# redmod-team/SympGPR

Hardware: AMD Instinct MI355X
Metric: Gram-build GB/s + Cholesky fp64 TFLOP/s at N=65536 d=2; |alpha-alpha_ref|/|alpha_ref| (higher is better)
Workload: dtype f64

## Files before the change

include/sympgpr_probe.h:

```cpp
#ifndef SYMPGPR_PROBE_H
#define SYMPGPR_PROBE_H
#include <stddef.h>
#ifdef __cplusplus
extern "C" {
#endif

int sgpr_probe_mfma_f64(int waves_per_simd, int iters, double *tflops);
int sgpr_probe_hbm_write(size_t bytes, int reps, double *gbs);
int sgpr_probe_mfma_clock(int nacc, int waves_per_simd, int iters, double *out3);
int sgpr_probe_gemm(int m, int n, int k, int lower, double *out4);
int sgpr_probe_gemm_debug(int bits);
int sgpr_probe_leaf(double *out8);
int sgpr_probe_lat(double *out8);
int sgpr_probe_xcc(int nblocks, int *host_out);
int sgpr_probe_cumask(const unsigned *mask_words, int nwords, int nblocks, int *host_out);

int sgpr_probe_generated_eval(int family, int which, int m, const double *xa, const double *ya,
                              const double *xb, const double *yb, const double *l, int nl, double *out);

int sgpr_probe_queue_plan(int n, int nworkers, int *starts_out, int max_starts, unsigned *tasks_out, int max_tasks,
                          int *counts);
int sgpr_probe_queue_plan_partial(int n, int nworkers, int nq, int *starts_out, int max_starts, unsigned *tasks_out,
                                  int max_tasks, int *counts);
int sgpr_probe_queue_trace_begin(int max_tasks);
int sgpr_probe_queue_trace_end(unsigned long long *out, int max_tasks);
int sgpr_probe_queue_trace_clear(void);
int sgpr_probe_queue_postmortem(int always);
int sgpr_probe_queue_force_giveup(int on);
int sgpr_probe_tune(const char *name, double value);
unsigned sgpr_probe_map_calls(void);
int sgpr_probe_map_team(int ntest, int n0);

int sgpr_probe_trsm_piece(int ticket, int cap, int strips, int out[5]);
int sgpr_probe_trsm_counts(int strips, int cap, unsigned long long out[2]);

int sgpr_probe_census(int na, int threads_a, int lds_a, int spin_a, const unsigned *mask_a, int nwords_a,
                      int nb, int threads_b, int lds_b, int spin_b, const unsigned *mask_b, int nwords_b,
                      unsigned long long *host_out);

#ifdef __cplusplus
}
#endif
#endif
```

sympgpr_amd/_lib.py:

```python
import ctypes as C
import os

import numpy as np

FAMILIES = {"A": 0, "B": 1, "C": 2, "D": 3, "USER": 4}
K_KERN, K_DXDX0, K_DYDY0, K_DXDY0 = 0, 1, 2, 3
K_DLX, K_DLY = 4, 8
K_DX, K_DY, K_DX0, K_DY0, K_DXDX0DY0, K_DYDY0DY0, K_DXDY0DY0 = 16, 17, 18, 19, 20, 21, 22
G_QQ, G_PQ, G_QP, G_PP, G_ALL, G_LOWER, G_OCML, G_DLX, G_DLY = 1, 2, 4, 8, 15, 16, 32, 64, 128
FIT_LOWER_ONLY, FIT_REG, FIT_BLOCK_QQ, FIT_BLOCK_PP = 1, 4, 8, 16
MAP_WRAP_Q, MAP_WRAP_P, MAP_EXPLICIT, MAP_LOSS_NEGP = 1, 2, 4, 8
E_ARG, E_NODEVICE, E_HIP, E_NOMEM, E_STATE = -1, -2, -3, -4, -5

ABI_VERSION = 5
_dp = C.POINTER(C.c_double)
_vp = C.c_void_p


class SympGPRError(RuntimeError):
    pass


class NoDeviceError(SympGPRError):
    pass
# ... 108 lines not shown
    "sgpr_probe_generated_eval": (C.c_int, [C.c_int, C.c_int, C.c_int, _dp, _dp, _dp, _dp, _dp, C.c_int, _dp]),
    "sgpr_probe_queue_plan": (C.c_int, [C.c_int, C.c_int, C.POINTER(C.c_int), C.c_int, C.POINTER(C.c_uint), C.c_int,
                                        C.POINTER(C.c_int)]),
    "sgpr_probe_queue_plan_partial": (C.c_int, [C.c_int, C.c_int, C.c_int, C.POINTER(C.c_int), C.c_int, C.POINTER(C.c_uint),
                                                C.c_int, C.POINTER(C.c_int)]),
    "sgpr_probe_queue_trace_begin": (C.c_int, [C.c_int]),
    "sgpr_probe_queue_trace_end": (C.c_int, [C.POINTER(C.c_ulonglong), C.c_int]),
    "sgpr_probe_queue_postmortem": (C.c_int, [C.c_int]),
    "sgpr_probe_queue_force_giveup": (C.c_int, [C.c_int]),
    "sgpr_probe_tune": (C.c_int, [C.c_char_p, C.c_double]),
    "sgpr_probe_map_calls": (C.c_uint, []),
    "sgpr_probe_map_team": (C.c_int, [C.c_int, C.c_int]),
    "sgpr_probe_trsm_piece": (C.c_int, [C.c_int, C.c_int, C.c_int, C.POINTER(C.c_int)]),
    "sgpr_probe_trsm_counts": (C.c_int, [C.c_int, C.c_int, C.POINTER(C.c_ulonglong)]),
    "sgpr_probe_queue_trace_clear": (C.c_int, []),
    "sgpr_probe_census": (C.c_int, [C.c_int, C.c_int, C.c_int, C.c_int, C.POINTER(C.c_uint), C.c_int,
                                    C.c_int, C.c_int, C.c_int, C.c_int, C.POINTER(C.c_uint), C.c_int,
                                    C.POINTER(C.c_ulonglong)]),
}

_LIB = None
_PROBE = None


def load_library():
    global _LIB
    if _LIB is not None:
        return _LIB
    path = lib_path()
    if os.environ.get("SYMPGPR_NO_TORCH_PRELOAD") != "1":
# ... 81 lines not shown
```

sympgpr_amd/csrc/chol.hip:

```cpp
#include <algorithm>
#include <cstdlib>
#include <mutex>
#include <vector>

#include "cholq.h"
#include "common.h"
#include "gemm_tile.h"
#include "leaf.h"

namespace sgpr {

namespace {

using namespace leaf;


__global__ __launch_bounds__(LT) void leaf_kernel(int nb, double *A, size_t lda, double *inv,
                                                  int *dinfo, int goff, int mode,
                                                  unsigned long long *stamps)
{
    __shared__ double s[LEAF_LDS];
    if (nb == LEAF) leaf_body(s, (int)LEAF, A, lda, inv, dinfo, goff, mode, stamps);
    else            leaf_body(s, nb, A, lda, inv, dinfo, goff, mode, stamps);
}
// ... 759 lines not shown

inline int split(int n)
{
    int n1 = ((n / 2 + LEAF - 1) / LEAF) * LEAF;
    if (n1 >= n) n1 -= LEAF;
    return n1;
}

struct Ctx {
    double *inv;
    int *dinfo;
    hipStream_t st;
    int la_max = 0;
    int *flags = nullptr;
    void *qws = nullptr;
};

int potrf_lookahead(int n, double *A, size_t lda, const Ctx &c, int nb, int off0);
inline int la_block(int n) { return n <= 4096 ? 256 : (n <= 24576 ? 512 : (n <= 40960 ? 1024 : 2048)); }

int trsm_rec(int m, int n, const double *L, size_t ldl, double *B, size_t ldb, int off, const Ctx &c)
{
    if (n <= LEAF) {
        return gemm_nt(m, n, n, 1.0, B, ldb, c.inv + (size_t)(off / LEAF) * LEAF * LEAF, LEAF, 0.0,
                       B, ldb, 0, 0, c.st);
    }
    const int n1 = split(n), n2 = n - n1;
    int rc = trsm_rec(m, n1, L, ldl, B, ldb, off, c);
    if (rc) return rc;
    rc = gemm_nt(m, n2, n1, -1.0, B, ldb, L + n1, ldl, 1.0, B + (size_t)n1 * ldb, ldb, 0, 0, c.st);
    if (rc) return rc;
    return trsm_rec(m, n2, L + n1 + (size_t)n1 * ldl, ldl, B + (size_t)n1 * ldb, ldb, off + n1, c);
}

int trsm_rl_rec(int m, int n, const double *L, size_t ldl, double *B, size_t ldb, int off, const Ctx &c)
{
    if (n <= LEAF)
        return gemm_nn(m, n, n, 1.0, B, ldb, c.inv + (size_t)(off / LEAF) * LEAF * LEAF, LEAF, 0.0, B, ldb, c.st);
    const int n1 = split(n), n2 = n - n1;
    int rc = trsm_rl_rec(m, n2, L + n1 + (size_t)n1 * ldl, ldl, B + (size_t)n1 * ldb, ldb, off + n1, c);
    if (rc) return rc;
    rc = gemm_nn(m, n1, n2, -1.0, B + (size_t)n1 * ldb, ldb, L + n1, ldl, 1.0, B, ldb, c.st);
    if (rc) return rc;
    return trsm_rl_rec(m, n1, L, ldl, B, ldb, off, c);
}
// ... 2 lines not shown
{
    if (n <= LEAF) {
        hipLaunchKernelGGL(leaf_kernel, dim3(1), dim3(LT), 0, c.st, n, A, lda,
                           c.inv + (size_t)(off / LEAF) * LEAF * LEAF, c.dinfo, off, (int)LEAF_FACTOR,
                           (unsigned long long *)nullptr);
        SGPR_CHECK_LAUNCH();
        return 0;
    }
    if (n > 4 * LEAF && n <= c.la_max) return potrf_lookahead(n, A, lda, c, 0, off);
    const int n1 = split(n), n2 = n - n1;
    double *A21 = A + n1, *A22 = A + n1 + (size_t)n1 * lda;
    int rc = potrf_rec(n1, A, lda, off, c);
    if (rc) return rc;
    rc = trsm_rec(n2, n1, A, lda, A21, lda, off, c);
    if (rc) return rc;
    rc = gemm_nt(n2, n2, n1, -1.0, A21, lda, A21, lda, 1.0, A22, lda, 1, 0, c.st);
    if (rc) return rc;
    return potrf_rec(n2, A22, lda, off + n1, c);
}

int trsv_n_rec(int n, const double *L, size_t ldl, double *b, int off, const Ctx &c)
{
    if (n <= LEAF) {
        hipLaunchKernelGGL(leaf_matvec_kernel, dim3(1), dim3(MV_T), 0, c.st, n,
                           c.inv + (size_t)(off / LEAF) * LEAF * LEAF, b, 0);
        SGPR_CHECK_LAUNCH();
        return 0;
    }
    if (n <= TRSV_BLOCK) {
        hipLaunchKernelGGL(trsv_block_kernel, dim3(1), dim3(MV_T), 0, c.st, n, L, ldl,
                           c.inv + (size_t)(off / LEAF) * LEAF * LEAF, b, 0);
// ... 560 lines not shown
    QueueDevice &qd = g_qdev[dev];
    std::lock_guard<std::mutex> lock(qd.mu);
    qd.failed = true;
    return true;
}

int potrf_trim()
{
    for (int dev = 0; dev < 64; ++dev) {
        EventPool &p = t_event_pool[dev];
        if (p.ev.empty() || p.top != 0) continue;
        for (hipEvent_t e : p.ev) (void)hipEventDestroy(e);
        p.ev.clear();
    }
    (void)hipGetLastError();
    return 0;
}

int release_device_streams(int dev)
{
    if (dev < 0 || dev >= 64) { set_error("release_device_streams: device index out of range"); return SGPR_E_ARG; }
    return release_streams(dev);
}

int potrf(int n, double *A, size_t lda, void *work, size_t lwork, int *dinfo, hipStream_t st)
{
    if (n < 0 || (n > 0 && lda < (size_t)n)) { set_error("potrf: bad n / lda"); return SGPR_E_ARG; }
    if (lwork < potrf_workspace(n)) { set_error("potrf: workspace too small"); return SGPR_E_ARG; }
    SGPR_HIP(hipMemsetAsync(dinfo, 0, sizeof(int), st));
    if (n == 0) return 0;
    int *flags = reinterpret_cast<int *>(static_cast<char *>(work) + inv_bytes(n));
    SGPR_HIP(hipMemsetAsync(flags, 0, flag_bytes(n), st));
    static const int mode = [] { const char *e = getenv("SGPR_POTRF"); return !e ? 0 : (e[0] == 'r' ? 1 : 2); }();
    static const int nb_env = [] { const char *e = getenv("SGPR_POTRF_NB"); return e ? atoi(e) : 0; }();
    static const int la_max_env = [] { const char *e = getenv("SGPR_LA_MAX"); return e ? atoi(e) : 57344; }();
    t_last_potrf_used_queue = false;
    Ctx c{static_cast<double *>(work), dinfo, st, mode == 1 ? 0 : la_max_env, flags};
    if (cholq::ws_bytes(n) > 0) c.qws = static_cast<char *>(work) + inv_bytes(n) + flag_bytes(n) + pub_bytes(n);
    const bool dbg = PANEL_DBG && getenv("SGPR_PANEL_DBG") != nullptr;
    const int T = (n + LEAF - 1) / LEAF;
    if (dbg) {
        (void)hipMalloc((void **)&g_panel_dbg, sizeof(unsigned long long) * 16 * T);
        (void)hipMemset(g_panel_dbg, 0, sizeof(unsigned long long) * 16 * T);
    }
    int rc;
    if (mode == 2 || (nb_env > 0 && mode == 0 && n > 4 * LEAF && n <= c.la_max))
        rc = potrf_lookahead(n, A, lda, c, nb_env > 0 ? nb_env : 0, 0);
    else
        rc = potrf_rec(n, A, lda, 0, c);
    if (dbg) {
        (void)hipStreamSynchronize(st);
        std::vector<unsigned long long> h(16 * (size_t)T);
        (void)hipMemcpy(h.data(), g_panel_dbg, h.size() * 8, hipMemcpyDeviceToHost);
// ... 171 lines not shown
```

sympgpr_amd/csrc/common.h:

```cpp
#pragma once
#include <hip/hip_runtime.h>
#include <cstddef>
#include <cstdint>
#include <string>

#include "../../include/sympgpr_hip.h"

namespace sgpr {

void set_error(const std::string &msg);
double tune(const char *name, double dflt);
void tune_set(const char *name, double v);
int hip_fail(hipError_t e, const char *what, const char *file, int line);

#define SGPR_HIP(call)                                                          \
    do {                                                                        \
        hipError_t e__ = (call);                                                \
        if (e__ != hipSuccess) return ::sgpr::hip_fail(e__, #call, __FILE__, __LINE__); \
    } while (0)

#define SGPR_CHECK_LAUNCH() SGPR_HIP(hipGetLastError())

struct KConst {
    double lx, ly, p, sig;
// ... 37 lines not shown
            const double *hyp, int nhyp, double *K, size_t ld, size_t rstride, size_t cstride, long diag_off,
            double noise, hipStream_t st);
int gram_nd_sel(int family, int d, int mi, int mj, const double *Xb, size_t ldxb, const double *Xa, size_t ldxa,
                const double *hyp, int nhyp, double *K, size_t ld, const long *roff, const long *coff, hipStream_t st);
int predict_nd(int family, int d, int m, const double *Xt, size_t ldxt, int n0, const double *Xtr, size_t ldxtr,
               const double *hyp, int nhyp, const double *alpha, double *out, hipStream_t st);

int gemm_nt(int m, int n, int k, double alpha, const double *A, size_t lda, const double *B,
            size_t ldb, double beta, double *C, size_t ldc, int lower, long diag_off,
            hipStream_t st);
int gemm_nt_bc(int m, int n, int k, double alpha, const double *A, size_t lda, const double *B,
               size_t ldb, double beta, double *C, size_t ldc, int lower, const int *bc5,
               hipStream_t st);
int gemm_nn(int m, int n, int k, double alpha, const double *A, size_t lda, const double *B, size_t ldb,
            double beta, double *C, size_t ldc, hipStream_t st);
int gemm_profile_begin();
int gemm_profile_end(double *out12);
int gemm_profile_launches(double *buf, int max_records);
void gemm_set_overlap(int on);
int gemm_nt_diag(int m, int n, int k, double alpha, const double *A, size_t lda, const double *B, size_t ldb,
                 double beta, double *C, size_t ldc, int lower, unsigned long long *stamps, int dbg, hipStream_t st);

constexpr int LEAF = 128;
constexpr int POTRF_HANDOFF_TIMEOUT = -1000001;
constexpr int SOLVE_HANDOFF_TIMEOUT = -1000002;
inline int info_status(int info)
{
    if (info >= 0) return info;
    set_error(info == POTRF_HANDOFF_TIMEOUT ? "potrf: a hand-off inside the panel kernel timed out"
              : info == SOLVE_HANDOFF_TIMEOUT ? "solve: a hand-off between the strips of a triangular solve timed out" : "potrf: internal error");
// ... 87 lines not shown
```

sympgpr_amd/csrc/gemm_f64.hip:

```cpp
#include <algorithm>
#include <atomic>
#include <cstdlib>
#include <mutex>
#include <type_traits>
#include <vector>

#include "common.h"
#include "gemm_tile.h"

namespace sgpr {

namespace {

struct ProfRec { double flop; int big; int m, n, k, lower, overlap; };
struct Prof {
    std::mutex mu;
    std::atomic<bool> on{false};
    std::vector<hipEvent_t> pool;
    std::vector<ProfRec> recs;
    long dropped = 0;
};
constexpr int PROF_POOL = 8192;
Prof g_prof;
thread_local int t_overlap = 0;
// ... 15 lines not shown
    }
    const bool aligned = ((((uintptr_t)g.A | (uintptr_t)g.B) & 15) == 0) && (((g.lda | g.ldb) & 1) == 0);
    const bool fast = aligned && (row0 + BM <= g.m) && (col0 + BN <= g.n) && (g.k % BK == 0);
    if (g.transb) {
        if (fast) gemm_body<BM, BN, true, true>(g, smem, tile_r, tile_c);
        else      gemm_body<BM, BN, false, true>(g, smem, tile_r, tile_c);
        return;
    }
    if constexpr (BM % 128 == 0) {
        if (fast && !(g.dbg & 16)) { gemm_body_dma<BM, BN, STAGES>(g, smem, tile_r, tile_c); return; }
    }
    if (fast) gemm_body<BM, BN, true>(g, smem, tile_r, tile_c);
    else      gemm_body<BM, BN, false>(g, smem, tile_r, tile_c);
}

}

int gemm_nt(int m, int n, int k, double alpha, const double *A, size_t lda, const double *B,
            size_t ldb, double beta, double *C, size_t ldc, int lower, long diag_off,
            hipStream_t st)
{
    const int bc[5] = {1, 1, (int)diag_off, 1, 0};
    return gemm_nt_bc(m, n, k, alpha, A, lda, B, ldb, beta, C, ldc, lower, bc, st);
}

static int gemm_launch(int m, int n, int k, double alpha, const double *A, size_t lda, const double *B,
                       size_t ldb, double beta, double *C, size_t ldc, int lower, const int *bc, int transb,
                       hipStream_t st, unsigned long long *stamps = nullptr, int dbg = 0);

int gemm_nt_bc(int m, int n, int k, double alpha, const double *A, size_t lda, const double *B,
               size_t ldb, double beta, double *C, size_t ldc, int lower, const int *bc,
               hipStream_t st)
{
    static const int kmax = [] { const char *e = getenv("SGPR_GEMM_KMAX"); return e ? atoi(e) : 8192; }();
    if (kmax >= 128 && k > kmax) {
        const int nchunk = (k + kmax - 1) / kmax;
        const int step = ((k + nchunk - 1) / nchunk + 127) / 128 * 128;
        for (int k0 = 0; k0 < k; k0 += step) {
            const int rc = gemm_launch(m, n, std::min(step, k - k0), alpha, A + (size_t)k0 * lda, lda, B + (size_t)k0 * ldb, ldb,
                                       k0 == 0 ? beta : 1.0, C, ldc, lower, bc, 0, st);
            if (rc) return rc;
        }
        return 0;
    }
    return gemm_launch(m, n, k, alpha, A, lda, B, ldb, beta, C, ldc, lower, bc, 0, st);
}

static int gemm_launch(int m, int n, int k, double alpha, const double *A, size_t lda, const double *B,
                       size_t ldb, double beta, double *C, size_t ldc, int lower, const int *bc, int transb,
                       hipStream_t st, unsigned long long *stamps, int dbg)
{
    const bool plain = bc[0] == 1 && bc[1] == 1 && bc[3] == 1 && bc[4] == 0;
    const long diag_off = plain ? bc[2] : 1;
    if (bc[0] < 1 || bc[1] < 1 || bc[3] < 1) { set_error("gemm_nt: bad block-cyclic descriptor"); return SGPR_E_ARG; }
    if (m < 0 || n < 0 || k < 0) { set_error("gemm_nt: negative extent"); return SGPR_E_ARG; }
    if (m == 0 || n == 0) return 0;
    if (lda < (size_t)m || ldb < (size_t)(transb ? k : n) || ldc < (size_t)m) {
        set_error("gemm: leading dimension too small");
        return SGPR_E_ARG;
    }
    GemmArgs g{m, n, k, alpha, beta, A, lda, B, ldb, C, ldc, lower, diag_off, transb, stamps, 0, 0, 0, 0, 0, 0,
               0, 0, bc[0], bc[1], bc[2], bc[3], bc[4], dbg};
    auto set_map = [&](int bm, int bn) {
        g.tiles_m = (m + bm - 1) / bm;
        g.tiles_n = (n + bn - 1) / bn;
        const int SC = (SR * bm) / (4 * bn);
        g.n_sr = (g.tiles_m + SR - 1) / SR;
        g.n_sc = (g.tiles_n + SC - 1) / SC;
        g.tri = (lower && diag_off == 0 && m == n) ? 1 : 0;
        if (g.tri) {
            long full = 0;
            for (int sc = 0; sc < g.n_sc; ++sc) full += std::max(g.n_sr - sc / 4 - 1, 0);
            g.n_full = (int)full;
            g.n_grp = (g.n_sc + 3) / 4;
            g.n_super = g.n_full + 4 * g.n_grp;
        }
        if (!g.tri) g.n_super = g.n_sr * g.n_sc;
// ... 28 lines not shown
                rec.flop = 2.0 * k * elems;
                rec.m = m; rec.n = n; rec.k = k; rec.lower = lower; rec.overlap = t_overlap;
                slot = (int)g_prof.recs.size();
                g_prof.recs.push_back(rec);
            } else {
                ++g_prof.dropped;
            }
        }
    }
    if (slot >= 0) SGPR_HIP(hipEventRecord(g_prof.pool[2 * slot], st));
    const long big = (long)((m + 255) / 256) * ((n + 127) / 128);
    static const bool prefer_big = tune("gemm_small_tile", 0) == 0;
    static const double small_mb = tune("gemm_small_mb", 0.0);
    const double op_bytes = 8.0 * (double)k * ((A == B && lda == ldb) ? (double)std::max(m, n) : (double)m + n);
    const bool small_k = op_bytes <= small_mb * 1e6 && m > 128 && n > 128;
    if (n <= 128 && m <= 32768 && !(dbg & 8)) {
        const dim3 grid(set_map(64, 128));
        hipLaunchKernelGGL((gemm_nt_kernel<64, 128>), grid, dim3(128), 0, st, g);
    } else if (prefer_big && !(dbg & 8) && !small_k && (big >= 256 || (m >= 256 && n == 128))) {
        const dim3 grid(set_map(256, 128));
        hipLaunchKernelGGL((gemm_nt_kernel<256, 128>), grid, dim3(512), 0, st, g);
        rec.big = 1;
    } else {
        const dim3 grid(set_map(128, 128));
        hipLaunchKernelGGL((gemm_nt_kernel<128, 128>), grid, dim3(256), 0, st, g);
    }
    SGPR_CHECK_LAUNCH();
    if (slot >= 0) {
        SGPR_HIP(hipEventRecord(g_prof.pool[2 * slot + 1], st));
        if (rec.big) {
            std::lock_guard<std::mutex> lock(g_prof.mu);
// ... 61 lines not shown
    for (size_t i = 0; i < g_prof.recs.size(); ++i) {
        const ProfRec &r = g_prof.recs[i];
        SGPR_HIP(hipEventSynchronize(g_prof.pool[2 * i + 1]));
        float ms = 0.f;
        SGPR_HIP(hipEventElapsedTime(&ms, g_prof.pool[2 * i], g_prof.pool[2 * i + 1]));
        const int o = r.big ? (r.overlap ? 8 : 0) : 3;
        out[o] += 1.0; out[o + 1] += r.flop; out[o + 2] += ms;
        if (r.flop > out[6]) { out[6] = r.flop; out[7] = ms; }
        for (double v : {(double)r.m, (double)r.n, (double)r.k, (double)r.lower, (double)r.big, (double)ms, (double)r.overlap})
            g_last_launches.push_back(v);
    }
    g_prof.recs.clear();
    return 0;
}

}
```

sympgpr_amd/csrc/gemm_tile.h:

```cpp
#pragma once
#include <type_traits>

#include "common.h"

namespace sgpr {
namespace tile {

typedef double double4_t __attribute__((ext_vector_type(4)));
typedef double double2_t __attribute__((ext_vector_type(2)));

#ifndef SGPR_GEMM_STAGES
#define SGPR_GEMM_STAGES 2
#endif
constexpr int BK = 16;
constexpr int PAD = 16;

struct GemmArgs {
    int m, n, k;
    double alpha, beta;
    const double *A;
    size_t lda;
    const double *B;
    size_t ldb;
    double *C;
    size_t ldc;
    int lower;
    long diag_off;
    int transb;
    unsigned long long *stamps;
    int tiles_m, tiles_n, n_sr, n_sc, n_super, tri;
    int n_full, n_grp;
    int lblk, lpr, lpi, lpc, lpj;
    int dbg;
    unsigned long long *kdone;
};

constexpr int SR = 8;
template <int SC>
__device__ __forceinline__ bool tile_of(const GemmArgs &g, int &tile_r, int &tile_c)
{
    const int L = blockIdx.x;
    const int xcd = L & 7, j = L >> 3;
    const int S = (j / (SR * SC)) * 8 + xcd;
    if (S >= g.n_super) return false;
    const int w = j % (SR * SC);
    int sr, sc;
    if (!g.tri) {
        sc = S / g.n_sr;
        sr = S - sc * g.n_sr;
// ... 95 lines not shown
    const int kp = 2 * (e % (BK / 2));
    const int r = e / (BK / 2);
    S[kp * (BR + PAD) + r] = v.x;
    S[(kp + 1) * (BR + PAD) + r] = v.y;
}

template <int BR, int THREADS>
__device__ __forceinline__ void store_pass(double *S, int tid, const double2_t &v, int p)
{
    const int e = p * THREADS + tid;
    const int r = 2 * (e % (BR / 2));
    const int kc = e / (BR / 2);
    *reinterpret_cast<double2_t *>(S + kc * (BR + PAD) + r) = v;
}

template <int BM, int BN, bool FAST, bool TRANSB = false>
__device__ __forceinline__ void gemm_body(const GemmArgs &g, double *smem, int tile_r, int tile_c)
{
    constexpr int WGM = BM / 64, WGN = BN / 64;
    constexpr int THREADS = 64 * WGM * WGN;
    constexpr int LDA_S = BM + PAD, LDB_S = BN + PAD;
    constexpr int PA = BM * BK / (2 * THREADS), PB = BN * BK / (2 * THREADS);
    static_assert(PA >= 1 && PB >= 1, "tile too small for the thread count");
    double *const sA0 = smem;
    double *const sB0 = smem + 2 * BK * LDA_S;
    const int row0 = tile_r * BM;
    const int col0 = tile_c * BN;

    const int tid = threadIdx.x;
    const int lane = tid & 63;
    const int wave = tid >> 6;
// ... 111 lines not shown
        __builtin_amdgcn_sched_barrier(0);
#pragma unroll
        for (int r = 0; r < 4; ++r) {
            const int n = col0 + wn * 64 + i * 16 + 4 * r + l4;
#pragma unroll
            for (int j = 0; j < 4; ++j) {
                const int m = row0 + wm * 64 + j * 16 + l15;
                if (interior || (m < g.m && n < g.n)) {
                    const double v = alpha * acc[i][j][r];
                    g.C[(size_t)m + (size_t)n * g.ldc] = (beta == 0.0) ? v : __builtin_fma(beta, old[r][j], v);
                }
            }
        }
        __builtin_amdgcn_sched_barrier(0);
    }
}

__device__ __forceinline__ unsigned lds_addr(const void *p)
{
    return (unsigned)(size_t)(const __attribute__((address_space(3))) void *)p;
}
template <int OFF>
__device__ __forceinline__ double ds_read_f64(unsigned addr)
{
    double v;
    asm volatile("ds_read_b64 %0, %1 offset:%2" : "=v"(v) : "v"(addr), "n"(OFF));
    return v;
}
template <int KK, int LDA_S, int LDB_S>
__device__ __forceinline__ void read_frags(unsigned aA, unsigned aB, double (&fa)[4], double (&fb)[4])
{
    fa[0] = ds_read_f64<(KK * 4 * LDB_S + 0) * 8>(aB);
    fb[0] = ds_read_f64<(KK * 4 * LDA_S + 0) * 8>(aA);
    fa[1] = ds_read_f64<(KK * 4 * LDB_S + 16) * 8>(aB);
    fb[1] = ds_read_f64<(KK * 4 * LDA_S + 16) * 8>(aA);
    fa[2] = ds_read_f64<(KK * 4 * LDB_S + 32) * 8>(aB);
    fb[2] = ds_read_f64<(KK * 4 * LDA_S + 32) * 8>(aA);
    fa[3] = ds_read_f64<(KK * 4 * LDB_S + 48) * 8>(aB);
    fb[3] = ds_read_f64<(KK * 4 * LDA_S + 48) * 8>(aA);
}
#define SGPR_LGKM_WAIT(n) do { asm volatile("s_waitcnt lgkmcnt(" #n ")" ::: "memory"); __builtin_amdgcn_sched_barrier(0); } while (0)

template <int BM, int BN, int STAGES>
__device__ __forceinline__ void gemm_body_dma(const GemmArgs &g, double *smem, int tile_r, int tile_c)
{
    constexpr int WGM = BM / 64, WGN = BN / 64;
    constexpr int NW = WGM * WGN;
    constexpr int LDA_S = BM + PAD, LDB_S = BN + PAD;
    constexpr int QA = BK * (BM / 128) / NW, QB = BK * (BN / 128) / NW;
    static_assert(QA >= 1 && QB >= 1 && BM % 128 == 0 && BN % 128 == 0, "tile / wave count mismatch");
    static_assert(STAGES == 2 || STAGES == 3, "two or three LDS stages");
    double *const sA0 = smem;
    double *const sB0 = smem + STAGES * BK * LDA_S;
    const int row0 = tile_r * BM, col0 = tile_c * BN;
    const int tid = threadIdx.x;
    const int lane = tid & 63;
    const int wave = __builtin_amdgcn_readfirstlane(tid >> 6);
    const int wm = wave % WGM, wn = wave / WGM;
// ... 143 lines not shown
        __builtin_amdgcn_sched_barrier(0);
        if (beta != 0.0) {
            if (i + 1 < 4) asm volatile("s_waitcnt vmcnt(16)" ::: "memory");
            else           asm volatile("s_waitcnt vmcnt(0)" ::: "memory");
        }
        __builtin_amdgcn_sched_barrier(0);
#pragma unroll
        for (int r = 0; r < 4; ++r)
#pragma unroll
            for (int j = 0; j < 4; ++j) {
                const double v = alpha * acc[i][j][r];
                cbase[(size_t)(j * 16) + (size_t)(i * 16 + 4 * r) * g.ldc] = (beta == 0.0) ? v : __builtin_fma(beta, old[i & 1][r][j], v);
            }
        __builtin_amdgcn_sched_barrier(0);
    }
}


}
}
```

sympgpr_amd/csrc/probe.hip:

```cpp
#include <algorithm>
#include <cstdlib>
#include <vector>

#include "cholq.h"
#include "common.h"
#include "../../include/sympgpr_probe.h"
#include "generated/pair_generated.h"

namespace sgpr {
namespace {
typedef double double4_t __attribute__((ext_vector_type(4)));
typedef double double2_t __attribute__((ext_vector_type(2)));

template <int NACC>
__global__ __launch_bounds__(256) void mfma_clock_kernel(int iters, double *out, unsigned long long *stamps)
{
    double4_t acc[NACC];
    const double a = 1.0 + threadIdx.x * 1e-9, b = 1.0 - threadIdx.x * 1e-9;
#pragma unroll
    for (int i = 0; i < NACC; ++i) acc[i] = double4_t{0.0, 0.0, 0.0, 0.0};
    const unsigned long long t0 = __builtin_amdgcn_s_memtime(), r0 = __builtin_amdgcn_s_memrealtime();
    for (int it = 0; it < iters; ++it) {
#pragma unroll
        for (int i = 0; i < NACC; ++i)
// ... 463 lines not shown
    const size_t words = cholq::trace_words((size_t)g_qtrace_cap);
    SGPR_HIP(hipMemcpy(out, g_qtrace, sizeof(unsigned long long) * words, hipMemcpyDeviceToHost));
    (void)hipFree(g_qtrace);
    g_qtrace = nullptr;
    return (int)words;
}

extern "C" int sgpr_probe_queue_postmortem(int always) { return cholq::postmortem(always != 0); }
extern "C" int sgpr_probe_queue_force_giveup(int on) { cholq::force_giveup(on); return 0; }
extern "C" int sgpr_probe_tune(const char *name, double value)
{
    if (!name) { set_error("probe_tune: null name"); return SGPR_E_ARG; }
    tune_set(name, value);
    return 0;
}
extern "C" unsigned sgpr_probe_map_calls(void) { return applymap_last_calls(); }
extern "C" int sgpr_probe_map_team(int ntest, int n0) { return applymap_team(ntest, n0); }
extern "C" int sgpr_probe_trsm_piece(int ticket, int cap, int strips, int out[5]) { if (ticket < 0 || cap < 1 || strips < 0 || !out) return SGPR_E_ARG; trsm_piece_of(ticket, cap, strips, out); return 0; }
extern "C" int sgpr_probe_trsm_counts(int strips, int cap, unsigned long long out[2])
{
    if (strips < 0 || cap < 1 || !out) return SGPR_E_ARG;
    size_t c[2];
    trsm_piece_counts(strips, cap, c);
    out[0] = c[0]; out[1] = c[1];
    return 0;
}

namespace sgpr { namespace {
__global__ void census_kernel(unsigned long long *out, int spin_us)
{
// ... 44 lines not shown
```

Before: 71.40.

## Use one-level Strassen for large trailing GEMM/SYRK updates in recursive Cholesky

Adds a Strassen-Winograd path for the large NT GEMM and SYRK trailing updates in the recursive potrf and trsm. Each Strassen level replaces eight half-size block products with seven. A new dual-output GEMM kernel writes each product into two C blocks, and block-sum kernels form the operand sums in a reserved scratch buffer. The aim is to cut fp64 MFMA work at N=65536, at the cost of extra memory traffic, scratch allocation and some accuracy loss. The path applies only to the top-level recursive split above la_max, because half-extents must be at least 8192.

Result: faster. 76.83 (median of 6 runs) (+7.6%).

```diff
diff --git a/include/sympgpr_probe.h b/include/sympgpr_probe.h
--- a/include/sympgpr_probe.h
+++ b/include/sympgpr_probe.h
@@ -28,6 +28,12 @@
 int sgpr_probe_queue_postmortem(int always);
 int sgpr_probe_queue_force_giveup(int on);
 int sgpr_probe_tune(const char *name, double value);
+int sgpr_probe_strassen_plan(int m, int n, int k, int lower, long smin, long kslab, long scratch_doubles, long long *out,
+                             int max_records, int *count);
+int sgpr_probe_gemm_strassen_dev(int m, int n, int k, double alpha, const double *A, size_t lda, const double *B, size_t ldb,
+                                 double beta, double *C, size_t ldc, int lower, void *stream);
+int sgpr_probe_gemm_nt2_dev(int m, int n, int k, double alpha, const double *A, size_t lda, const double *B, size_t ldb,
+                            double beta, double *C, size_t ldc, double alpha2, double *C2, size_t ldc2, void *stream);
 unsigned sgpr_probe_map_calls(void);
 int sgpr_probe_map_team(int ntest, int n0);
 
diff --git a/sympgpr_amd/_lib.py b/sympgpr_amd/_lib.py
--- a/sympgpr_amd/_lib.py
+++ b/sympgpr_amd/_lib.py
@@ -146,6 +146,12 @@
     "sgpr_probe_trsm_piece": (C.c_int, [C.c_int, C.c_int, C.c_int, C.POINTER(C.c_int)]),
     "sgpr_probe_trsm_counts": (C.c_int, [C.c_int, C.c_int, C.POINTER(C.c_ulonglong)]),
     "sgpr_probe_queue_trace_clear": (C.c_int, []),
+    "sgpr_probe_strassen_plan": (C.c_int, [C.c_int, C.c_int, C.c_int, C.c_int, C.c_long, C.c_long, C.c_long,
+                                           C.POINTER(C.c_longlong), C.c_int, C.POINTER(C.c_int)]),
+    "sgpr_probe_gemm_strassen_dev": (C.c_int, [C.c_int, C.c_int, C.c_int, C.c_double, C.c_void_p, C.c_size_t, C.c_void_p, C.c_size_t,
+                                               C.c_double, C.c_void_p, C.c_size_t, C.c_int, C.c_void_p]),
+    "sgpr_probe_gemm_nt2_dev": (C.c_int, [C.c_int, C.c_int, C.c_int, C.c_double, C.c_void_p, C.c_size_t, C.c_void_p, C.c_size_t,
+                                          C.c_double, C.c_void_p, C.c_size_t, C.c_double, C.c_void_p, C.c_size_t, C.c_void_p]),
     "sgpr_probe_census": (C.c_int, [C.c_int, C.c_int, C.c_int, C.c_int, C.POINTER(C.c_uint), C.c_int,
                                     C.c_int, C.c_int, C.c_int, C.c_int, C.POINTER(C.c_uint), C.c_int,
                                     C.POINTER(C.c_ulonglong)]),
diff --git a/sympgpr_amd/csrc/chol.hip b/sympgpr_amd/csrc/chol.hip
--- a/sympgpr_amd/csrc/chol.hip
+++ b/sympgpr_amd/csrc/chol.hip
@@ -797,6 +797,7 @@
     int la_max = 0;
     int *flags = nullptr;
     void *qws = nullptr;
+    bool strassen = false;
 };
 
 int potrf_lookahead(int n, double *A, size_t lda, const Ctx &c, int nb, int off0);
@@ -811,7 +812,8 @@
     const int n1 = split(n), n2 = n - n1;
     int rc = trsm_rec(m, n1, L, ldl, B, ldb, off, c);
     if (rc) return rc;
-    rc = gemm_nt(m, n2, n1, -1.0, B, ldb, L + n1, ldl, 1.0, B + (size_t)n1 * ldb, ldb, 0, 0, c.st);
+    if (c.strassen) rc = gemm_nt_strassen(m, n2, n1, -1.0, B, ldb, L + n1, ldl, 1.0, B + (size_t)n1 * ldb, ldb, 0, c.st);
+    else            rc = gemm_nt(m, n2, n1, -1.0, B, ldb, L + n1, ldl, 1.0, B + (size_t)n1 * ldb, ldb, 0, 0, c.st);
     if (rc) return rc;
     return trsm_rec(m, n2, L + n1 + (size_t)n1 * ldl, ldl, B + (size_t)n1 * ldb, ldb, off + n1, c);
 }
@@ -844,7 +846,8 @@
     if (rc) return rc;
     rc = trsm_rec(n2, n1, A, lda, A21, lda, off, c);
     if (rc) return rc;
-    rc = gemm_nt(n2, n2, n1, -1.0, A21, lda, A21, lda, 1.0, A22, lda, 1, 0, c.st);
+    if (c.strassen) rc = gemm_nt_strassen(n2, n2, n1, -1.0, A21, lda, A21, lda, 1.0, A22, lda, 1, c.st);
+    else            rc = gemm_nt(n2, n2, n1, -1.0, A21, lda, A21, lda, 1.0, A22, lda, 1, 0, c.st);
     if (rc) return rc;
     return potrf_rec(n2, A22, lda, off + n1, c);
 }
@@ -1435,7 +1438,7 @@
         p.ev.clear();
     }
     (void)hipGetLastError();
-    return 0;
+    return strassen_trim();
 }
 
 int release_device_streams(int dev)
@@ -1454,10 +1457,15 @@
     SGPR_HIP(hipMemsetAsync(flags, 0, flag_bytes(n), st));
     static const int mode = [] { const char *e = getenv("SGPR_POTRF"); return !e ? 0 : (e[0] == 'r' ? 1 : 2); }();
     static const int nb_env = [] { const char *e = getenv("SGPR_POTRF_NB"); return e ? atoi(e) : 0; }();
-    static const int la_max_env = [] { const char *e = getenv("SGPR_LA_MAX"); return e ? atoi(e) : 57344; }();
+    static const int la_max_env = [] { const char *e = getenv("SGPR_LA_MAX"); return (int)tune("la_max", e ? atoi(e) : 57344); }();
     t_last_potrf_used_queue = false;
     Ctx c{static_cast<double *>(work), dinfo, st, mode == 1 ? 0 : la_max_env, flags};
     if (cholq::ws_bytes(n) > 0) c.qws = static_cast<char *>(work) + inv_bytes(n) + flag_bytes(n) + pub_bytes(n);
+    c.strassen = true;
+    if (n > c.la_max && n > LEAF) {
+        const int n1 = split(n), n2 = n - n1, n11 = split(n1);
+        strassen_reserve(std::max(strassen_scratch_doubles(n2, n2, n1, 1), strassen_scratch_doubles(n2, n1 - n11, n11, 0)), st);
+    }
     const bool dbg = PANEL_DBG && getenv("SGPR_PANEL_DBG") != nullptr;
     const int T = (n + LEAF - 1) / LEAF;
     if (dbg) {
diff --git a/sympgpr_amd/csrc/common.h b/sympgpr_amd/csrc/common.h
--- a/sympgpr_amd/csrc/common.h
+++ b/sympgpr_amd/csrc/common.h
@@ -3,6 +3,7 @@
 #include <cstddef>
 #include <cstdint>
 #include <string>
+#include <vector>
 
 #include "../../include/sympgpr_hip.h"
 
@@ -75,6 +76,16 @@
                hipStream_t st);
 int gemm_nn(int m, int n, int k, double alpha, const double *A, size_t lda, const double *B, size_t ldb,
             double beta, double *C, size_t ldc, hipStream_t st);
+int gemm_nt_two(int m, int n, int k, double alpha, const double *A, size_t lda, const double *B, size_t ldb, double beta,
+             double *C, size_t ldc, double alpha2, double *C2, size_t ldc2, hipStream_t st);
+constexpr int STRASSEN_REC = 16;
+enum { PLAN_SUM = 1, PLAN_PROD = 2, PLAN_CLASSIC = 3 };
+int gemm_nt_strassen(int m, int n, int k, double alpha, const double *A, size_t lda, const double *B, size_t ldb, double beta,
+                     double *C, size_t ldc, int lower, hipStream_t st);
+int strassen_plan(int m, int n, int k, int lower, long smin, long kslab, size_t scratch_doubles, std::vector<long long> &out);
+size_t strassen_scratch_doubles(int m, int n, int k, int lower);
+void strassen_reserve(size_t doubles, hipStream_t st);
+int strassen_trim();
 int gemm_profile_begin();
 int gemm_profile_end(double *out12);
 int gemm_profile_launches(double *buf, int max_records);
diff --git a/sympgpr_amd/csrc/gemm_f64.hip b/sympgpr_amd/csrc/gemm_f64.hip
--- a/sympgpr_amd/csrc/gemm_f64.hip
+++ b/sympgpr_amd/csrc/gemm_f64.hip
@@ -53,6 +53,43 @@
     else      gemm_body<BM, BN, false>(g, smem, tile_r, tile_c);
 }
 
+__global__ __launch_bounds__(512, 2) void gemm_nt2_kernel(const GemmArgs g)
+{
+    constexpr int BM = 256, BN = 128, LDA_S = BM + PAD, LDB_S = BN + PAD;
+    __shared__ double smem[SGPR_GEMM_STAGES * BK * (LDA_S + LDB_S)];
+    int tile_r, tile_c;
+    if (!tile_of<(SR * BM) / (4 * BN)>(g, tile_r, tile_c)) return;
+    const int row0 = tile_r * BM, col0 = tile_c * BN;
+    const bool aligned = ((((uintptr_t)g.A | (uintptr_t)g.B) & 15) == 0) && (((g.lda | g.ldb) & 1) == 0);
+    const bool fast = aligned && (row0 + BM <= g.m) && (col0 + BN <= g.n) && (g.k % BK == 0);
+    if (fast) gemm_body_dma<BM, BN, SGPR_GEMM_STAGES, true>(g, smem, tile_r, tile_c);
+    else      gemm_body<BM, BN, false, false, true>(g, smem, tile_r, tile_c);
+}
+
+__global__ __launch_bounds__(256) void block_sum_kernel(int rows, int cols, const double *X, size_t ldx, const double *Y, size_t ldy,
+                                                        double sign, double *T)
+{
+    const int nrc = (rows + 511) / 512, ncg = (cols + 3) / 4;
+    const long pieces = (long)nrc * ncg;
+    for (long p = blockIdx.x; p < pieces; p += gridDim.x) {
+        const int cg = (int)(p / nrc), rc = (int)(p - (long)cg * nrc);
+        const int r = rc * 512 + 2 * (int)threadIdx.x;
+        if (r >= rows) continue;
+        double2_t x[4], y[4];
+#pragma unroll
+        for (int u = 0; u < 4; ++u) {
+            const int c = min(cg * 4 + u, cols - 1);
+            x[u] = *reinterpret_cast<const double2_t *>(X + (size_t)r + (size_t)c * ldx);
+            y[u] = *reinterpret_cast<const double2_t *>(Y + (size_t)r + (size_t)c * ldy);
+        }
+#pragma unroll
+        for (int u = 0; u < 4; ++u) {
+            const int c = cg * 4 + u;
+            if (c < cols) *reinterpret_cast<double2_t *>(T + (size_t)r + (size_t)c * (size_t)rows) = x[u] + sign * y[u];
+        }
+    }
+}
+
 }
 
 int gemm_nt(int m, int n, int k, double alpha, const double *A, size_t lda, const double *B,
@@ -65,11 +102,12 @@
 
 static int gemm_launch(int m, int n, int k, double alpha, const double *A, size_t lda, const double *B,
                        size_t ldb, double beta, double *C, size_t ldc, int lower, const int *bc, int transb,
-                       hipStream_t st, unsigned long long *stamps = nullptr, int dbg = 0);
-
-int gemm_nt_bc(int m, int n, int k, double alpha, const double *A, size_t lda, const double *B,
-               size_t ldb, double beta, double *C, size_t ldc, int lower, const int *bc,
-               hipStream_t st)
+                       hipStream_t st, unsigned long long *stamps = nullptr, int dbg = 0, double *C2 = nullptr,
+                       size_t ldc2 = 0, double alpha2 = 0.0);
+
+static int gemm_chunked(int m, int n, int k, double alpha, const double *A, size_t lda, const double *B,
+                        size_t ldb, double beta, double *C, size_t ldc, int lower, const int *bc,
+                        hipStream_t st, double *C2, size_t ldc2, double alpha2)
 {
     static const int kmax = [] { const char *e = getenv("SGPR_GEMM_KMAX"); return e ? atoi(e) : 8192; }();
     if (kmax >= 128 && k > kmax) {
@@ -77,17 +115,32 @@
         const int step = ((k + nchunk - 1) / nchunk + 127) / 128 * 128;
         for (int k0 = 0; k0 < k; k0 += step) {
             const int rc = gemm_launch(m, n, std::min(step, k - k0), alpha, A + (size_t)k0 * lda, lda, B + (size_t)k0 * ldb, ldb,
-                                       k0 == 0 ? beta : 1.0, C, ldc, lower, bc, 0, st);
+                                       k0 == 0 ? beta : 1.0, C, ldc, lower, bc, 0, st, nullptr, 0, C2, ldc2, alpha2);
             if (rc) return rc;
         }
         return 0;
     }
-    return gemm_launch(m, n, k, alpha, A, lda, B, ldb, beta, C, ldc, lower, bc, 0, st);
+    return gemm_launch(m, n, k, alpha, A, lda, B, ldb, beta, C, ldc, lower, bc, 0, st, nullptr, 0, C2, ldc2, alpha2);
+}
+
+int gemm_nt_bc(int m, int n, int k, double alpha, const double *A, size_t lda, const double *B,
+               size_t ldb, double beta, double *C, size_t ldc, int lower, const int *bc,
+               hipStream_t st)
+{
+    return gemm_chunked(m, n, k, alpha, A, lda, B, ldb, beta, C, ldc, lower, bc, st, nullptr, 0, 0.0);
+}
+
+int gemm_nt_two(int m, int n, int k, double alpha, const double *A, size_t lda, const double *B, size_t ldb, double beta,
+             double *C, size_t ldc, double alpha2, double *C2, size_t ldc2, hipStream_t st)
+{
+    const int bc[5] = {1, 1, 0, 1, 0};
+    if (!C2) { set_error("gemm_nt_two: null second destination"); return SGPR_E_ARG; }
+    return gemm_chunked(m, n, k, alpha, A, lda, B, ldb, beta, C, ldc, 0, bc, st, C2, ldc2, alpha2);
 }
 
 static int gemm_launch(int m, int n, int k, double alpha, const double *A, size_t lda, const double *B,
                        size_t ldb, double beta, double *C, size_t ldc, int lower, const int *bc, int transb,
-                       hipStream_t st, unsigned long long *stamps, int dbg)
+                       hipStream_t st, unsigned long long *stamps, int dbg, double *C2, size_t ldc2, double alpha2)
 {
     const bool plain = bc[0] == 1 && bc[1] == 1 && bc[3] == 1 && bc[4] == 0;
     const long diag_off = plain ? bc[2] : 1;
@@ -98,8 +151,9 @@
         set_error("gemm: leading dimension too small");
         return SGPR_E_ARG;
     }
+    if (C2 && (lower || transb || ldc2 < (size_t)m)) { set_error("gemm: bad second destination"); return SGPR_E_ARG; }
     GemmArgs g{m, n, k, alpha, beta, A, lda, B, ldb, C, ldc, lower, diag_off, transb, stamps, 0, 0, 0, 0, 0, 0,
-               0, 0, bc[0], bc[1], bc[2], bc[3], bc[4], dbg};
+               0, 0, bc[0], bc[1], bc[2], bc[3], bc[4], dbg, nullptr, C2, ldc2, alpha2};
     auto set_map = [&](int bm, int bn) {
         g.tiles_m = (m + bm - 1) / bm;
         g.tiles_n = (n + bn - 1) / bn;
@@ -158,7 +212,11 @@
     static const double small_mb = tune("gemm_small_mb", 0.0);
     const double op_bytes = 8.0 * (double)k * ((A == B && lda == ldb) ? (double)std::max(m, n) : (double)m + n);
     const bool small_k = op_bytes <= small_mb * 1e6 && m > 128 && n > 128;
-    if (n <= 128 && m <= 32768 && !(dbg & 8)) {
+    if (C2) {
+        const dim3 grid(set_map(256, 128));
+        hipLaunchKernelGGL(gemm_nt2_kernel, grid, dim3(512), 0, st, g);
+        rec.big = 1;
+    } else if (n <= 128 && m <= 32768 && !(dbg & 8)) {
         const dim3 grid(set_map(64, 128));
         hipLaunchKernelGGL((gemm_nt_kernel<64, 128>), grid, dim3(128), 0, st, g);
     } else if (prefer_big && !(dbg & 8) && !small_k && (big >= 256 || (m >= 256 && n == 128))) {
@@ -250,4 +308,240 @@
     return 0;
 }
 
-}
+namespace {
+struct PlanCfg {
+    long smin;
+    long kslab;
+    size_t scratch;
+};
+void put(std::vector<long long> &out, std::initializer_list<long long> v)
+{
+    size_t i = 0;
+    for (long long x : v) { out.push_back(x); ++i; }
+    for (; i < STRASSEN_REC; ++i) out.push_back(0);
+}
+long slab_of(long k, const PlanCfg &c)
+{
+    if (k <= 0 || k % 32 != 0 || c.kslab < 32) return 0;
+    const long nslab = (k + c.kslab - 1) / c.kslab;
+    const long step = ((k + nslab - 1) / nslab + 31) / 32 * 32;
+    const long kmin = std::max(c.smin / 2, 16L);
+    const long last = k - (nslab - 1) * step;
+    if (last <= 0 || step / 2 < kmin || last / 2 < kmin) return 0;
+    return step;
+}
+bool qualifies(long m, long n, long k, const PlanCfg &c)
+{
+    if (m <= 0 || n <= 0 || m % 512 != 0 || n % 256 != 0) return false;
+    if (m / 2 < c.smin || n / 2 < c.smin) return false;
+    const long step = slab_of(k, c);
+    if (!step) return false;
+    return (size_t)(m / 2 + n / 2) * (size_t)(step / 2) <= c.scratch;
+}
+void plan_gemm(long m, long n, long k, long ar, long br, long cr, long cc, const PlanCfg &c, std::vector<long long> &out)
+{
+    if (!qualifies(m, n, k, c)) {
+        put(out, {PLAN_CLASSIC, 0, ar, 0, br, 0, m, n, k, cr, cc});
+        return;
+    }
+    const long m2 = m / 2, n2 = n / 2, step = slab_of(k, c);
+    for (long k0 = 0; k0 < k; k0 += step) {
+        const long k2 = std::min(step, k - k0) / 2;
+        const long a1 = ar, a2 = ar + m2, b1 = br, b2 = br + n2, j1 = k0, j2 = k0 + k2;
+        const long c1r = cr, c2r = cr + m2, c1c = cc, c2c = cc + n2;
+        auto sum = [&](int side, long xr, long xc, long yr, long yc, int sign) {
+            put(out, {PLAN_SUM, side, side ? n2 : m2, k2, xr, xc, yr, yc, sign});
+        };
+        auto prod = [&](int as, long pr, long pc, int bs, long qr, long qc, long d1r, long d1c, int s1, long d2r, long d2c, int s2) {
+            put(out, {PLAN_PROD, as, pr, pc, bs, qr, qc, m2, n2, k2, d1r, d1c, s1, d2r, d2c, s2});
+        };
+        sum(0, a1, j1, a2, j2, +1); sum(1, b1, j1, b2, j2, +1);
+        prod(1, 0, 0, 1, 0, 0, c1r, c1c, +1, c2r, c2c, +1);
+        sum(0, a2, j1, a2, j2, +1);
+        prod(1, 0, 0, 0, b1, j1, c2r, c1c, +1, c2r, c2c, -1);
+        sum(1, b2, j1, b2, j2, -1);
+        prod(0, a1, j1, 1, 0, 0, c1r, c2c, +1, c2r, c2c, +1);
+        sum(1, b1, j2, b1, j1, -1);
+        prod(0, a2, j2, 1, 0, 0, c1r, c1c, +1, c2r, c1c, +1);
+        sum(0, a1, j1, a1, j2, +1);
+        prod(1, 0, 0, 0, b2, j2, c1r, c1c, -1, c1r, c2c, +1);
+        sum(0, a2, j1, a1, j1, -1); sum(1, b1, j1, b2, j1, +1);
+        prod(1, 0, 0, 1, 0, 0, c2r, c2c, +1, 0, 0, 0);
+        sum(0, a1, j2, a2, j2, -1); sum(1, b1, j2, b2, j2, +1);
+        prod(1, 0, 0, 1, 0, 0, c1r, c1c, +1, 0, 0, 0);
+    }
+}
+void plan_syrk(long n, long k, long r0, const PlanCfg &c, std::vector<long long> &out)
+{
+    const long h = n / 2;
+    if (n % 2 != 0 || !qualifies(h, h, k, c)) {
+        put(out, {PLAN_CLASSIC, 1, r0, 0, r0, 0, n, n, k, r0, r0});
+        return;
+    }
+    plan_syrk(h, k, r0, c, out);
+    plan_gemm(h, h, k, r0 + h, r0, r0 + h, r0, c, out);
+    plan_syrk(h, k, r0 + h, c, out);
+}
+size_t plan_need(const std::vector<long long> &plan)
+{
+    size_t need[2] = {0, 0};
+    for (size_t i = 0; i + STRASSEN_REC <= plan.size(); i += STRASSEN_REC)
+        if (plan[i] == PLAN_SUM) need[plan[i + 1]] = std::max(need[plan[i + 1]], (size_t)plan[i + 2] * (size_t)plan[i + 3]);
+    return need[0] + need[1];
+}
+
+bool strassen_on()
+{
+    static const bool on = [] { const char *e = getenv("SGPR_GEMM_STRASSEN"); return !(e && e[0] == '0'); }();
+    return on;
+}
+PlanCfg default_cfg()
+{
+    static const long smin = std::max(128L, (long)tune("gemm_strassen_min", 8192));
+    static const long kslab = std::max(32L, (long)tune("gemm_strassen_kslab", 16384));
+    return PlanCfg{smin, kslab, ~(size_t)0};
+}
+
+struct Scratch {
+    std::mutex mu;
+    double *p = nullptr;
+    size_t cap = 0, failed = 0;
+    hipEvent_t ev = nullptr;
+    hipStream_t last = nullptr;
+    bool used = false;
+};
+Scratch g_scratch[64];
+
+bool scratch_ensure(Scratch &s, size_t need)
+{
+    static const bool forced_fail = tune("gemm_strassen_noscratch", 0) != 0;
+    if (forced_fail) return false;
+    if (s.cap >= need) return true;
+    if (s.failed && need >= s.failed) return false;
+    if (s.p) { (void)hipFree(s.p); s.p = nullptr; s.cap = 0; s.used = false; }
+    if (hipMalloc((void **)&s.p, need * sizeof(double)) != hipSuccess) {
+        (void)hipGetLastError();
+        s.p = nullptr;
+        s.failed = need;
+        return false;
+    }
+    s.cap = need;
+    return true;
+}
+int device_of(hipStream_t st)
+{
+    int dev = -1;
+    if ((st ? hipStreamGetDevice(st, &dev) : hipGetDevice(&dev)) != hipSuccess) { (void)hipGetLastError(); return -1; }
+    return (dev >= 0 && dev < 64) ? dev : -1;
+}
+
+int block_sum(int rows, int cols, const double *X, size_t ldx, const double *Y, size_t ldy, double sign, double *T, hipStream_t st)
+{
+    const long pieces = (long)((rows + 511) / 512) * ((cols + 3) / 4);
+    hipLaunchKernelGGL(block_sum_kernel, dim3((unsigned)std::min(pieces, 2048L)), dim3(256), 0, st, rows, cols, X, ldx, Y, ldy, sign, T);
+    SGPR_CHECK_LAUNCH();
+    return 0;
+}
+
+int run_plan(const std::vector<long long> &plan, double alpha, const double *A, size_t lda, const double *B, size_t ldb,
+             double beta, double *C, size_t ldc, double *SA, double *SB, hipStream_t st)
+{
+    for (size_t i = 0; i + STRASSEN_REC <= plan.size(); i += STRASSEN_REC) {
+        const long long *r = &plan[i];
+        int rc = 0;
+        if (r[0] == PLAN_SUM) {
+            const double *P = r[1] ? B : A;
+            const size_t ld = r[1] ? ldb : lda;
+            rc = block_sum((int)r[2], (int)r[3], P + r[4] + (size_t)r[5] * ld, ld, P + r[6] + (size_t)r[7] * ld, ld, (double)r[8],
+                           r[1] ? SB : SA, st);
+        } else if (r[0] == PLAN_PROD) {
+            const int m = (int)r[7], n = (int)r[8], k = (int)r[9];
+            const double *Ap = r[1] ? SA : A + r[2] + (size_t)r[3] * lda;
+            const double *Bp = r[4] ? SB : B + r[5] + (size_t)r[6] * ldb;
+            double *C1 = C + r[10] + (size_t)r[11] * ldc;
+            if (r[15]) rc = gemm_nt_two(m, n, k, alpha * (double)r[12], Ap, r[1] ? (size_t)m : lda, Bp, r[4] ? (size_t)n : ldb, 1.0, C1, ldc,
+                                     alpha * (double)r[15], C + r[13] + (size_t)r[14] * ldc, ldc, st);
+            else       rc = gemm_nt(m, n, k, alpha * (double)r[12], Ap, r[1] ? (size_t)m : lda, Bp, r[4] ? (size_t)n : ldb, 1.0, C1, ldc, 0, 0, st);
+        } else {
+            rc = gemm_nt((int)r[6], (int)r[7], (int)r[8], alpha, A + r[2] + (size_t)r[3] * lda, lda, B + r[4] + (size_t)r[5] * ldb, ldb,
+                         beta, C + r[9] + (size_t)r[10] * ldc, ldc, (int)r[1], 0, st);
+        }
+        if (rc) return rc;
+    }
+    return 0;
+}
+}
+
+int strassen_plan(int m, int n, int k, int lower, long smin, long kslab, size_t scratch_doubles, std::vector<long long> &out)
+{
+    if (m < 0 || n < 0 || k < 0 || (lower && m != n)) { set_error("strassen_plan: bad extents"); return SGPR_E_ARG; }
+    PlanCfg c = default_cfg();
+    if (smin >= 0) c.smin = std::max(128L, smin);
+    if (kslab >= 0) c.kslab = std::max(32L, kslab);
+    c.scratch = scratch_doubles;
+    out.clear();
+    if (lower) plan_syrk(n, k, 0, c, out);
+    else       plan_gemm(m, n, k, 0, 0, 0, 0, c, out);
+    return 0;
+}
+
+size_t strassen_scratch_doubles(int m, int n, int k, int lower)
+{
+    std::vector<long long> plan;
+    if (!strassen_on() || strassen_plan(m, n, k, lower, -1, -1, ~(size_t)0, plan)) return 0;
+    return plan_need(plan);
+}
+
+void strassen_reserve(size_t doubles, hipStream_t st)
+{
+    const int dev = device_of(st);
+    if (!doubles || dev < 0 || !strassen_on()) return;
+    Scratch &s = g_scratch[dev];
+    std::lock_guard<std::mutex> lock(s.mu);
+    (void)scratch_ensure(s, doubles);
+}
+
+int strassen_trim()
+{
+    for (Scratch &s : g_scratch) {
+        std::lock_guard<std::mutex> lock(s.mu);
+        if (s.p) (void)hipFree(s.p);
+        if (s.ev) (void)hipEventDestroy(s.ev);
+        s.p = nullptr; s.ev = nullptr; s.cap = 0; s.failed = 0; s.used = false; s.last = nullptr;
+    }
+    (void)hipGetLastError();
+    return 0;
+}
+
+int gemm_nt_strassen(int m, int n, int k, double alpha, const double *A, size_t lda, const double *B, size_t ldb, double beta,
+                     double *C, size_t ldc, int lower, hipStream_t st)
+{
+    const bool aligned = ((((uintptr_t)A | (uintptr_t)B) & 15) == 0) && (((lda | ldb) & 1) == 0);
+    if (std::min(m, n) / 2 < default_cfg().smin || !strassen_on() || !aligned || beta != 1.0 || (lower && m != n))
+        return gemm_nt(m, n, k, alpha, A, lda, B, ldb, beta, C, ldc, lower, 0, st);
+    std::vector<long long> plan;
+    int rc = strassen_plan(m, n, k, lower, -1, -1, ~(size_t)0, plan);
+    if (rc) return rc;
+    const size_t need = plan_need(plan);
+    if (!need) return run_plan(plan, alpha, A, lda, B, ldb, beta, C, ldc, nullptr, nullptr, st);
+    const int dev = device_of(st);
+    if (dev < 0) return gemm_nt(m, n, k, alpha, A, lda, B, ldb, beta, C, ldc, lower, 0, st);
+    Scratch &s = g_scratch[dev];
+    std::lock_guard<std::mutex> lock(s.mu);
+    if (!scratch_ensure(s, need)) {
+        if ((rc = strassen_plan(m, n, k, lower, -1, -1, s.cap, plan))) return rc;
+        if (!plan_need(plan)) return run_plan(plan, alpha, A, lda, B, ldb, beta, C, ldc, nullptr, nullptr, st);
+    }
+    if (!s.ev) SGPR_HIP(hipEventCreateWithFlags(&s.ev, hipEventDisableTiming));
+    if (s.used && s.last != st) SGPR_HIP(hipStreamWaitEvent(st, s.ev, 0));
+    size_t na = 0;
+    for (size_t i = 0; i + STRASSEN_REC <= plan.size(); i += STRASSEN_REC)
+        if (plan[i] == PLAN_SUM && plan[i + 1] == 0) na = std::max(na, (size_t)plan[i + 2] * (size_t)plan[i + 3]);
+    rc = run_plan(plan, alpha, A, lda, B, ldb, beta, C, ldc, s.p, s.p + na, st);
+    SGPR_HIP(hipEventRecord(s.ev, st));
+    s.last = st;
+    s.used = true;
+    return rc;
+}
+
+}
diff --git a/sympgpr_amd/csrc/gemm_tile.h b/sympgpr_amd/csrc/gemm_tile.h
--- a/sympgpr_amd/csrc/gemm_tile.h
+++ b/sympgpr_amd/csrc/gemm_tile.h
@@ -33,6 +33,9 @@
     int lblk, lpr, lpi, lpc, lpj;
     int dbg;
     unsigned long long *kdone;
+    double *C2;
+    size_t ldc2;
+    double alpha2;
 };
 
 constexpr int SR = 8;
@@ -158,7 +161,7 @@
     *reinterpret_cast<double2_t *>(S + kc * (BR + PAD) + r) = v;
 }
 
-template <int BM, int BN, bool FAST, bool TRANSB = false>
+template <int BM, int BN, bool FAST, bool TRANSB = false, bool TWO = false>
 __device__ __forceinline__ void gemm_body(const GemmArgs &g, double *smem, int tile_r, int tile_c)
 {
     constexpr int WGM = BM / 64, WGN = BN / 64;
@@ -300,6 +303,34 @@
         }
         __builtin_amdgcn_sched_barrier(0);
     }
+    if constexpr (TWO) {
+        const double alpha2 = g.alpha2;
+#pragma unroll
+        for (int i = 0; i < 4; ++i) {
+            double old[4][4];
+#pragma unroll
+            for (int r = 0; r < 4; ++r) {
+                const int n = col0 + wn * 64 + i * 16 + 4 * r + l4;
+#pragma unroll
+                for (int j = 0; j < 4; ++j) {
+                    const int m = row0 + wm * 64 + j * 16 + l15;
+                    old[r][j] = (interior || (m < g.m && n < g.n)) ? g.C2[(size_t)m + (size_t)n * g.ldc2] : 0.0;
+                }
+            }
+            __builtin_amdgcn_sched_barrier(0);
+#pragma unroll
+            for (int r = 0; r < 4; ++r) {
+                const int n = col0 + wn * 64 + i * 16 + 4 * r + l4;
+#pragma unroll
+                for (int j = 0; j < 4; ++j) {
+                    const int m = row0 + wm * 64 + j * 16 + l15;
+                    if (interior || (m < g.m && n < g.n))
+                        g.C2[(size_t)m + (size_t)n * g.ldc2] = __builtin_fma(alpha2, acc[i][j][r], old[r][j]);
+                }
+            }
+            __builtin_amdgcn_sched_barrier(0);
+        }
+    }
 }
 
 __device__ __forceinline__ unsigned lds_addr(const void *p)
@@ -327,7 +358,7 @@
 }
 #define SGPR_LGKM_WAIT(n) do { asm volatile("s_waitcnt lgkmcnt(" #n ")" ::: "memory"); __builtin_amdgcn_sched_barrier(0); } while (0)
 
-template <int BM, int BN, int STAGES>
+template <int BM, int BN, int STAGES, bool TWO = false>
 __device__ __forceinline__ void gemm_body_dma(const GemmArgs &g, double *smem, int tile_r, int tile_c)
 {
     constexpr int WGM = BM / 64, WGN = BN / 64;
@@ -501,8 +532,33 @@
             }
         __builtin_amdgcn_sched_barrier(0);
     }
-}
-
-
-}
-}
+    if constexpr (TWO) {
+        const double alpha2 = g.alpha2;
+        double *const cbase2 = g.C2 + (size_t)(row0 + wm * 64 + l15) + (size_t)(col0 + wn * 64 + l4) * g.ldc2;
+        auto fetch2 = [&](int i, double (&o)[4][4]) {
+#pragma unroll
+            for (int r = 0; r < 4; ++r)
+#pragma unroll
+                for (int j = 0; j < 4; ++j) o[r][j] = cbase2[(size_t)(j * 16) + (size_t)(i * 16 + 4 * r) * g.ldc2];
+        };
+        fetch2(0, old[0]);
+#pragma unroll
+        for (int i = 0; i < 4; ++i) {
+            if (i + 1 < 4) fetch2(i + 1, old[(i + 1) & 1]);
+            __builtin_amdgcn_sched_barrier(0);
+            if (i + 1 < 4) asm volatile("s_waitcnt vmcnt(16)" ::: "memory");
+            else           asm volatile("s_waitcnt vmcnt(0)" ::: "memory");
+            __builtin_amdgcn_sched_barrier(0);
+#pragma unroll
+            for (int r = 0; r < 4; ++r)
+#pragma unroll
+                for (int j = 0; j < 4; ++j)
+                    cbase2[(size_t)(j * 16) + (size_t)(i * 16 + 4 * r) * g.ldc2] = __builtin_fma(alpha2, acc[i][j][r], old[i & 1][r][j]);
+            __builtin_amdgcn_sched_barrier(0);
+        }
+    }
+}
+
+
+}
+}
diff --git a/sympgpr_amd/csrc/probe.hip b/sympgpr_amd/csrc/probe.hip
--- a/sympgpr_amd/csrc/probe.hip
+++ b/sympgpr_amd/csrc/probe.hip
@@ -501,6 +501,28 @@
     tune_set(name, value);
     return 0;
 }
+
+extern "C" int sgpr_probe_strassen_plan(int m, int n, int k, int lower, long smin, long kslab, long scratch_doubles, long long *out,
+                                        int max_records, int *count)
+{
+    if (!count || scratch_doubles < 0) { set_error("probe_strassen_plan: bad arguments"); return SGPR_E_ARG; }
+    std::vector<long long> plan;
+    const int rc = strassen_plan(m, n, k, lower, smin, kslab, (size_t)scratch_doubles, plan);
+    if (rc) return rc;
+    *count = (int)(plan.size() / STRASSEN_REC);
+    for (size_t i = 0; out && i < plan.size() && (int)(i / STRASSEN_REC) < max_records; ++i) out[i] = plan[i];
+    return 0;
+}
+extern "C" int sgpr_probe_gemm_strassen_dev(int m, int n, int k, double alpha, const double *A, size_t lda, const double *B, size_t ldb,
+                                            double beta, double *C, size_t ldc, int lower, void *stream)
+{
+    return gemm_nt_strassen(m, n, k, alpha, A, lda, B, ldb, beta, C, ldc, lower, static_cast<hipStream_t>(stream));
+}
+extern "C" int sgpr_probe_gemm_nt2_dev(int m, int n, int k, double alpha, const double *A, size_t lda, const double *B, size_t ldb,
+                                       double beta, double *C, size_t ldc, double alpha2, double *C2, size_t ldc2, void *stream)
+{
+    return gemm_nt_two(m, n, k, alpha, A, lda, B, ldb, beta, C, ldc, alpha2, C2, ldc2, static_cast<hipStream_t>(stream));
+}
 extern "C" unsigned sgpr_probe_map_calls(void) { return applymap_last_calls(); }
 extern "C" int sgpr_probe_map_team(int ntest, int n0) { return applymap_team(ntest, n0); }
 extern "C" int sgpr_probe_trsm_piece(int ticket, int cap, int strips, int out[5]) { if (ticket < 0 || cap < 1 || strips < 0 || !out) return SGPR_E_ARG; trsm_piece_of(ticket, cap, strips, out); return 0; }
```
